# voletiv/mcvd-pytorch

Measured on AMD Instinct MI355X. Metric: sampled frames/sec (whole node), SMMNIST 64x64 DDPM 100-step, higher is better.
Workload: dtype f32-equivalent: f32 storage and accumulation; 58 of 58 3x3 convs, 41 of 41 1x1 convs and the attention products (head dims 32..128) as SIX bf16 piece products of operands split EXACTLY into three bf16 pieces (all 24 bits, fp32 exponent range, less than one fp32 rounding per product; tests/test_gpu_p

## Files before the change

mcvd_pytorch_amd/csrc/build.py:

```python
import argparse
import concurrent.futures as cf
import glob
import os
import subprocess
import sys

HERE = os.path.dirname(os.path.abspath(__file__))
PKG = os.path.dirname(HERE)
ROOT = os.path.dirname(PKG)
OBJ = os.path.join(HERE, "build")
LIB = os.path.join(PKG, "libmcvd_hip.so")
HIPCC = os.environ.get("HIPCC", "/opt/rocm/bin/hipcc")
FLAGS = ["--offload-arch=gfx950", "-O3", "-std=c++17", "-fPIC", "-Wall", "-Wno-unused-function",
         "-I", os.path.join(ROOT, "include")]
WINO_OBJS = ("conv_wino.o", "conv_wino3.o", "conv_wino2h.o", "conv_wino3p.o")
HOST_ONLY_FLAGS = {"model.cpp": ["-ffp-contract=off"], "api.cpp": ["-ffp-contract=off"],
                   "sampler.cpp": ["-ffp-contract=off"],
                   "dsm.cpp": ["-ffp-contract=off"],
                   "lpips.cpp": ["-ffp-contract=off"]}


def sources():
    return sorted(glob.glob(os.path.join(HERE, "*.cpp")) + glob.glob(os.path.join(HERE, "kernels", "*.cpp")))


def headers():
    return (glob.glob(os.path.join(HERE, "*.h")) + glob.glob(os.path.join(HERE, "kernels", "*.h"))
            + glob.glob(os.path.join(ROOT, "include", "*.h")) + [os.path.abspath(__file__)])


def compile_one(src, force, diag=False):
    obj = os.path.join(OBJ + ("_diag" if diag else ""), os.path.basename(src)[:-4] + ".o")
    newest_dep = max(os.path.getmtime(p) for p in [src] + headers())
    if not force and os.path.exists(obj) and os.path.getmtime(obj) >= newest_dep:
        return obj, None
    cmd = [HIPCC] + FLAGS + (["-DMCVD_DIAG"] if diag else []) + HOST_ONLY_FLAGS.get(os.path.basename(src), []) + ["-c", src, "-o", obj]
    r = subprocess.run(cmd, capture_output=True, text=True)
    if r.returncode != 0:
        raise RuntimeError("hipcc failed: %s\n%s" % (" ".join(cmd), r.stderr))
    return obj, r.stderr.strip()


def build(force=False, jobs=None, verbose=True, diag=False):
    lib = os.path.join(PKG, "libmcvd_hip_diag.so") if diag else LIB
    os.makedirs(OBJ + ("_diag" if diag else ""), exist_ok=True)
    srcs = sources()
    objs, rebuilt, wino_rebuilt = [], 0, False
    with cf.ThreadPoolExecutor(max_workers=jobs or os.cpu_count()) as ex:
        for obj, log in ex.map(lambda s: compile_one(s, force, diag), srcs):
            objs.append(obj)
            if log is not None:
                rebuilt += 1
                wino_rebuilt |= os.path.basename(obj) in WINO_OBJS
                if log and verbose:
                    print(log, file=sys.stderr)
    relink = rebuilt or not os.path.exists(lib) or force
    stamp = os.path.join(OBJ + ("_diag" if diag else ""), "wino_isa.ok")
    newest_wino = max(os.path.getmtime(os.path.join(OBJ + ("_diag" if diag else ""), o)) for o in WINO_OBJS)
    checked = os.path.exists(stamp) and os.path.getmtime(stamp) >= newest_wino
    if wino_rebuilt or (relink and not checked) or not checked:
        r = subprocess.run([sys.executable, os.path.join(ROOT, "tools", "check_wino_isa.py")] + (["--diag"] if diag else []),
                           capture_output=True, text=True)
        if r.returncode != 0:
            for o in WINO_OBJS:
                try:
                    os.remove(os.path.join(OBJ + ("_diag" if diag else ""), o))
                except OSError:
                    pass
            raise RuntimeError("Winograd kernels: generated code violates the asm-load invariants\n" + r.stderr)
        open(stamp, "w").write(r.stdout)
        if verbose:
            print(r.stdout.strip())
    if relink:
        cmd = [HIPCC, "--offload-arch=gfx950", "-shared", "-fPIC", "-o", lib] + objs + ["-ldl"]
        r = subprocess.run(cmd, capture_output=True, text=True)
        if r.returncode != 0:
            raise RuntimeError("link failed: %s\n%s" % (" ".join(cmd), r.stderr))
    if relink:
        r = subprocess.run([sys.executable, os.path.join(ROOT, "tools", "check_vop3p_dual_read.py"), lib], capture_output=True, text=True)
        if r.returncode != 0:
            os.remove(lib)
            raise RuntimeError("the library contains the gfx950 co-residency erratum form (write the affine with fma_unpacked, common.h)\n" + r.stdout + r.stderr)
        if verbose:
            print(r.stdout.strip())
    if verbose:
        print("%s: %d/%d objects rebuilt -> %s" % (os.path.basename(lib), rebuilt, len(srcs), lib))
    return lib


if __name__ == "__main__":
    ap = argparse.ArgumentParser()
    ap.add_argument("--force", action="store_true")
    ap.add_argument("-j", type=int, default=None)
    ap.add_argument("--diag", action="store_true", help="build libmcvd_hip_diag.so (-DMCVD_DIAG) instead")
    a = ap.parse_args()
    build(force=a.force, jobs=a.j, diag=a.diag)
```

mcvd_pytorch_amd/csrc/kernels/conv1x1_h2.cpp:

```cpp
#include <stdlib.h>

#include "../common.h"
#include "pieces.h"

namespace mcvd {

typedef float f32x16 __attribute__((ext_vector_type(16)));
typedef float f32x2 __attribute__((ext_vector_type(2)));
typedef unsigned u32x4 __attribute__((ext_vector_type(4)));

__device__ __forceinline__ float silu_q(float v) { return v * __builtin_amdgcn_rcpf(1.0f + __expf(-v)); }

constexpr int Q1_PT = 128;
constexpr int Q1_CK = 16;
constexpr int Q1_NB = 4;
constexpr int Q1_MAXIMG = 4;

template <int NP, int COT, int PRO, int EXP = 0, bool KV = false, bool IM = false>
__global__ __launch_bounds__(256, 2) void conv1x1_h2_kernel(ConvArgs a, int ptiles, int nct) {
    typedef Pieces<NP> PX;
    constexpr int PT = Q1_PT, CK = Q1_CK, NB = Q1_NB, BCO = 32 * COT;
    constexpr int PPR = PT / 4;
    constexpr int RPS = 256 / PPR;
    constexpr int XSZ = CK * PT;
    constexpr int WDW = COT * NP * 256;
    constexpr int WPC = WDW / 4;
    constexpr int MAXX = XSZ / 4 / 256;
    constexpr int MAXW = (WPC + 255) / 256;
    constexpr int G = (IM ? 0 : MAXX) + MAXW;
    static_assert(MAXX * 256 * 4 == XSZ && WPC % 64 == 0, "DMA rounds");
    extern __shared__ __attribute__((aligned(16))) float smem[];
    unsigned* sW = reinterpret_cast<unsigned*>(smem);
    float* sX = smem + NB * WDW;
    float* sC = sX + (IM ? 0 : NB * XSZ);

    const int tid = threadIdx.x, lane = tid & 63, wave = tid >> 6, l31 = lane & 31, half = lane >> 5;
    const int xcd = blockIdx.x & 7, slot = blockIdx.x >> 3;
    const int ptile = (slot / nct) * 8 + xcd, ctile = slot - (slot / nct) * nct;
    if (ptile >= ptiles) return;
    const int co0 = ctile * BCO;
    const int HW = a.H * a.W, Cin = a.Cin;
    const long NPX = (long)a.B * HW;
    const long gp0 = (long)ptile * PT;
    const int NS = a.CoutP / 32;

    long xg = gp0 + (tid % PPR) * 4;
    if (xg > NPX - 4) xg = NPX - 4;
    const int xb = (int)(xg / HW), xp = (int)(xg - (long)xb * HW);
    const int x_ci = tid / PPR;
    const int voff0 = (xb * a.C0 + x_ci) * HW + xp;
    const int voff1 = (xb * a.C1 + x_ci) * HW + xp;

    const unsigned* wbase = reinterpret_cast<const unsigned*>(NP == 2 ? a.wph : a.wpb) + PX::HDR + (long)ctile * COT * (NP * 256);
    const int wave_u = __builtin_amdgcn_readfirstlane(wave);
    int w_goff[MAXW], w_lds[MAXW];
#pragma unroll
    for (int s = 0; s < MAXW; ++s) {
        const int q0 = (s * 256 + wave_u * 64) % WPC;
        w_lds[s] = q0 * 4;
        w_goff[s] = (q0 + lane) * 4;
    }

    const int b_first = (int)(gp0 / HW);
    const int nimg = HW >= PT ? 1 : PT / HW;
    if (PRO != 0) {
        const int ppi = Cin >> 1;
        for (int q0 = 0; q0 < nimg * ppi; q0 += 256) {
            const int q = q0 + tid;
            if (q < nimg * ppi) {
                const int im = q / ppi, w = q - im * ppi;
                __builtin_amdgcn_global_load_lds(
                    (const __attribute__((address_space(1))) void*)(a.coef + ((long)min(b_first + im, a.B - 1) * Cin) * 2 + w * 4),
                    (__attribute__((address_space(3))) void*)(sC + (q0 + wave * 64) * 4), 16, 0, 0);
            }
        }
    }
    const int my_img = HW >= PT ? 0 : (wave * 32) / HW;
    const int x_lane = wave * 32 + l31 + half * PT;

#define Q1_DMA(ch)                                                                                              \
    {                                                                                                           \
        const int cb = (ch) * CK;                                                                               \
        const unsigned* wsrc = wbase + (long)(ch) * NS * (NP * 256);                                                  \
        unsigned* wdst = sW + ((ch) & (NB - 1)) * WDW;                                                          \
        _Pragma("unroll") for (int s = 0; s < MAXW; ++s)                                                        \
            __builtin_amdgcn_global_load_lds(                                                                   \
                (const __attribute__((address_space(1))) void*)(wsrc + w_goff[s]),                              \
                (__attribute__((address_space(3))) void*)(wdst + w_lds[s]), 16, 0, 0);                          \
        if constexpr (!IM) {                                                                                    \
            const bool second = cb >= a.C0;                                                                     \
            const float* xsrc = second ? a.x1 + (long)(cb - a.C0) * HW : a.x0 + (long)cb * HW;                  \
            const int voff = second ? voff1 : voff0;                                                            \
            float* xdst = sX + ((ch) & (NB - 1)) * XSZ;                                                         \
            _Pragma("unroll") for (int s = 0; s < MAXX; ++s)                                                    \
                __builtin_amdgcn_global_load_lds(                                                               \
                    (const __attribute__((address_space(1))) void*)(xsrc + (long)s * RPS * HW + voff),          \
                    (__attribute__((address_space(3))) void*)(xdst + (s * 256 + wave * 64) * 4), 16, 0, 0);     \
        }                                                                                                       \
    }

    f32x16 acc[COT];
#pragma unroll
    for (int ct = 0; ct < COT; ++ct)
#pragma unroll
        for (int r = 0; r < 16; ++r) acc[ct][r] = 0.0f;

    const bool rec = a.dbg != nullptr && wave == 0;
    unsigned long long tk0 = 0, tk1 = 0, tk2 = 0, rt0 = 0;
    if (rec) { rt0 = __builtin_amdgcn_s_memrealtime(); tk0 = __builtin_amdgcn_s_memtime(); }

    const int nchunks = Cin / CK;
    Q1_DMA(0);
    if (nchunks > 1) Q1_DMA(1);
    if (nchunks > 2) Q1_DMA(2);
    float* sPatch = sX;
    const int im_W = a.W, im_PR = PT / (IM ? a.W : PT) + 2, im_PITCH = a.W + 8, im_Cc = a.C0 + a.C1;
    const int im_plane = im_PR * im_PITCH;
    int* sTab = reinterpret_cast<int*>(sPatch + (im_Cc + 1) * im_plane);
    int im_base = 0;
    if constexpr (IM) {
        typedef float f4 __attribute__((ext_vector_type(4)));
        const int y0 = (int)((gp0 - (long)b_first * HW) / im_W);
        const int w4 = im_W >> 2, lw4 = 31 - __builtin_clz(w4);
        const int rows = (im_Cc + 1) * im_PR;
        for (int u0 = 0; u0 < rows * w4; u0 += 2 * 256) {
            f4 v[2];
            int dst[2];
#pragma unroll
            for (int j = 0; j < 2; ++j) {
                const int u = u0 + j * 256 + tid;
                const int row = u >> lw4, q = u & (w4 - 1);
                const int c = row / im_PR, ry = row - c * im_PR;
                const int yy = y0 - 1 + ry;
                v[j] = f4{0.0f, 0.0f, 0.0f, 0.0f};
                dst[j] = u < rows * w4 ? row * im_PITCH + 4 + 4 * q : -1;
                if (dst[j] >= 0 && c < im_Cc && yy >= 0 && yy < a.H)
                    v[j] = *reinterpret_cast<const f4*>(c < a.C0 ? a.x0 + (((long)b_first * a.C0 + c) * a.H + yy) * im_W + 4 * q
                                                                 : a.x1 + (((long)b_first * a.C1 + (c - a.C0)) * a.H + yy) * im_W + 4 * q);
            }
#pragma unroll
            for (int j = 0; j < 2; ++j)
                if (dst[j] >= 0) *reinterpret_cast<f4*>(sPatch + dst[j]) = v[j];
        }
        for (int u = tid; u < 2 * rows; u += 256)
            *reinterpret_cast<f4*>(sPatch + (u >> 1) * im_PITCH + (u & 1) * (im_W + 4)) = f4{0.0f, 0.0f, 0.0f, 0.0f};
        for (int kk = tid; kk < Cin; kk += 256) {
            const int c = kk / 9, t = kk - 9 * c;
            const int off = c < im_Cc ? c * im_plane + (t / 3) * im_PITCH + (t % 3) + 3 : im_Cc * im_plane + 4;
            sTab[(kk >> 4) * 16 + (kk & 1) * 8 + ((kk & 15) >> 1)] = off;
        }
        const int p = wave * 32 + l31;
        im_base = (p / im_W) * im_PITCH + (p % im_W);
    }
    if (rec) tk1 = __builtin_amdgcn_s_memtime();
#define Q1_STAGE(k, BV, CF)                                                                                     \
    {                                                                                                           \
        const int after = nchunks - 1 - (k);                                                                    \
        if (after >= 2) asm volatile("s_waitcnt vmcnt(%0)" :: "n"(2 * G) : "memory");                           \
        else if (after == 1) asm volatile("s_waitcnt vmcnt(%0)" :: "n"(G) : "memory");                          \
        else asm volatile("s_waitcnt vmcnt(0)" ::: "memory");                                                   \
        if (!(EXP & 8)) {       \
            asm volatile("" ::: "memory");                                                                      \
            __builtin_amdgcn_s_waitcnt(0xC07F);                                                  \
            __builtin_amdgcn_s_barrier();                                                                       \
            asm volatile("" ::: "memory");                                                                      \
        }                                                                                                       \
        if ((k) + 3 < nchunks && !(EXP & 1)) Q1_DMA((k) + 3);                                                   \
        const float* sXc = sX + ((k) & (NB - 1)) * XSZ + x_lane;        \
        const float* sCb = sC + ((long)my_img * Cin + (k) * CK) * 2 + half * 2;                                 \
        if constexpr (IM) {      \
            const u32x4* tp = reinterpret_cast<const u32x4*>(sTab + (k) * 16 + half * 8);                       \
            const u32x4 t0 = tp[0], t1 = tp[1];                                                                 \
            const float* pb = sPatch + im_base;                                                                 \
            BV[0] = pb[t0[0]]; BV[1] = pb[t0[1]]; BV[2] = pb[t0[2]]; BV[3] = pb[t0[3]];                         \
            BV[4] = pb[t1[0]]; BV[5] = pb[t1[1]]; BV[6] = pb[t1[2]]; BV[7] = pb[t1[3]];                         \
        } else {                                                                                                \
        _Pragma("unroll") for (int e = 0; e < 8; ++e) {          \
            BV[e] = sXc[2 * e * PT];                                                                            \
            if (PRO != 0) CF[e] = *reinterpret_cast<const f32x2*>(sCb + 4 * e);                                 \
        }                                                                                                       \
        }                                                                                                       \
        __builtin_amdgcn_sched_barrier(0);                                                                      \
    }
#define Q1_READ_AW(k, AW)                                                                                       \
    {                                                                                                           \
        const u32x4* sWc = reinterpret_cast<const u32x4*>(sW + ((k) & (NB - 1)) * WDW) + lane;                  \
        _Pragma("unroll") for (int ct = 0; ct < COT; ++ct)                                                      \
            _Pragma("unroll") for (int p = 0; p < NP; ++p) AW[ct][p] = sWc[(ct * NP + p) * 64];                 \
    }
#define Q1_PREP(BV, CF, BP)                                                                                     \
    if (EXP & 4) { _Pragma("unroll") for (int p = 0; p < NP; ++p) _Pragma("unroll") for (int j = 0; j < 4; ++j) BP[p][j] = __builtin_bit_cast(unsigned, BV[2 * j]); } else \
    {                                                                                                           \
        _Pragma("unroll") for (int e = 0; e < 8; ++e) {                                                         \
            if (PRO != 0) {      \
                asm("v_fma_f32 %0, %1, %2, %3" : "=v"(BV[e]) : "v"(BV[e]), "v"(CF[e].x), "v"(CF[e].y));         \
                if (PRO == 2) BV[e] = silu_q(BV[e]);                                                            \
            }                                                                                                   \
            if (NP == 2) BV[e] *= PX::ACT_SCALE;                                                                \
        }                                                                                                       \
        _Pragma("unroll") for (int j = 0; j < 4; ++j) {                                                         \
            unsigned w[NP];                                                                                     \
            PX::template split<false>(BV[2 * j], BV[2 * j + 1], w);                                             \
            _Pragma("unroll") for (int p = 0; p < NP; ++p) BP[p][j] = w[p];                                     \
        }                                                                                                       \
    }
#define Q1_MMA(AW, BP)                                                                                          \
    if (EXP & 2) { _Pragma("unroll") for (int ct = 0; ct < COT; ++ct) acc[ct][0] += __builtin_bit_cast(float, AW[ct][0][0] ^ BP[0][1] ^ AW[ct][NP - 1][2] ^ BP[NP - 1][3]); } else \
    {                                                                                                           \
        _Pragma("unroll") for (int k = 0; k < PX::NPROD; ++k)                                                   \
            _Pragma("unroll") for (int ct = 0; ct < COT; ++ct) acc[ct] = PX::mfma(AW[ct][PX::PA(k)], BP[PX::PB(k)], acc[ct]); \
    }
#define Q1_STEP(k, BPC, BPN)                                                                                    \
    {                                                                                                           \
        Q1_STAGE((k) + 1, bv, cf)                                                                               \
        Q1_MMA(aw, BPC)                                                                                         \
        Q1_PREP(bv, cf, BPN)                                                                                    \
         \
        if (!(EXP & 16)) {                                                                                      \
             \
            __builtin_amdgcn_sched_group_barrier(0x008, 3, 0);                                                  \
            _Pragma("unroll") for (int i_ = 3; i_ < PX::NPROD * COT; ++i_) {                                    \
                __builtin_amdgcn_sched_group_barrier(0x002, NVS, 0);                                            \
                __builtin_amdgcn_sched_group_barrier(0x008, 1, 0);                                              \
            }                                                                                                   \
            _Pragma("unroll") for (int p_ = 0; p_ < NP; ++p_) asm volatile("" : "+v"(BPN[p_]));                 \
        }                                                                                                       \
        Q1_READ_AW((k) + 1, aw)                                                                                 \
    }
    constexpr int NVS = (PRO == 2 ? 120 : PRO == 1 ? 76 : 64) / (PX::NPROD * COT > 3 ? PX::NPROD * COT - 3 : 1) + 1;
    {
        float bv[8];
        f32x2 cf[8];
        u32x4 aw[COT][NP], bpA[NP], bpB[NP];
        Q1_STAGE(0, bv, cf)
        Q1_READ_AW(0, aw)
        Q1_PREP(bv, cf, bpA)
        int ch = 0;
        for (; ch + 2 < nchunks; ch += 2) {
            Q1_STEP(ch, bpA, bpB)
            Q1_STEP(ch + 1, bpB, bpA)
        }
        if (ch + 1 < nchunks) {
            Q1_STEP(ch, bpA, bpB)
            Q1_MMA(aw, bpB)
        } else {
            Q1_MMA(aw, bpA)
        }
    }
#undef Q1_STEP
#undef Q1_STAGE
#undef Q1_READ_AW
#undef Q1_PREP
#undef Q1_MMA
#undef Q1_DMA
    if (rec) tk2 = __builtin_amdgcn_s_memtime();

    const float inv = NP == 2 ? a.wph[2] * (1.0f / PX::ACT_SCALE) : 1.0f;
    float* sO = smem;
    constexpr int OPT = PT + 4;
    typedef float f32x4 __attribute__((ext_vector_type(4)));
    const int px4 = tid & 31, cr = tid >> 5;
    const long gp = gp0 + px4 * 4;
    const bool valid = gp < NPX;
    const long gpc = valid ? gp : 0;
    const int ob = (int)(gpc / HW), op = (int)(gpc - (long)ob * HW);
    const long obase = (long)ob * a.Cout * HW + op;
    float e_bias[BCO / 8];
    f32x4 e_res[BCO / 8];
#pragma unroll
    for (int k = 0; k < BCO / 8; ++k) {
        const int co = co0 + cr + 8 * k;
        e_bias[k] = a.bias[co];
        e_res[k] = f32x4{0.0f, 0.0f, 0.0f, 0.0f};
        if (a.res) e_res[k] = *reinterpret_cast<const f32x4*>(a.res + obase + (long)min(co, a.Cout - 1) * HW);
    }
    asm volatile("s_waitcnt lgkmcnt(0)\n\ts_barrier" ::: "memory");
#pragma unroll
    for (int ct = 0; ct < COT; ++ct)
#pragma unroll
        for (int r = 0; r < 16; ++r)
            sO[(ct * 32 + (r & 3) + 8 * (r >> 2) + 4 * half) * OPT + wave * 32 + l31] = acc[ct][r] * inv;
    asm volatile("s_waitcnt lgkmcnt(0)\n\ts_barrier" ::: "memory");
    bool kv_tile[COT];
#pragma unroll
    for (int ct = 0; ct < COT; ++ct) kv_tile[ct] = false;
    if constexpr (KV) {
        const int Cq = a.kv_C, D = a.kv_D, DT = D >> 5, heads = Cq / D, ntl = HW >> 5;
        unsigned* img = reinterpret_cast<unsigned*>(a.kv_img);
#pragma unroll
        for (int ct = 0; ct < COT; ++ct) {
            const int cs = co0 + ct * 32;
            const int which = cs / Cq;
            if (which != 1 && which != 2) continue;
            kv_tile[ct] = true;
            const int within = cs - which * Cq, head = within / D, ch0 = within - head * D;
#pragma unroll
            for (int rnd = 0; rnd < 2; ++rnd) {
                const int item = rnd * 256 + tid;
                if (which == 1) {
                    const int rp = item >> 5, p4 = item & 31;
                    const int st_l = rp >> 3, j = (rp >> 1) & 3, h = rp & 1;
                    const int rl = ct * 32 + 16 * st_l + 4 * j + h;
                    const long g = gp0 + p4 * 4;
                    if (g < NPX) {
                        const int bb = (int)(g / HW), pix = (int)(g - (long)bb * HW);
                        const f32x4 v0 = *reinterpret_cast<const f32x4*>(sO + rl * OPT + p4 * 4) + a.bias[co0 + rl];
                        const f32x4 v1 = *reinterpret_cast<const f32x4*>(sO + (rl + 2) * OPT + p4 * 4) + a.bias[co0 + rl + 2];
                        unsigned w[4][3];
#pragma unroll
                        for (int i4 = 0; i4 < 4; ++i4) Pieces<3>::template split<false>(v0[i4], v1[i4], w[i4]);
                        const int st = (ch0 >> 4) + st_l;
                        unsigned* d1 = img + ((long)(bb * heads + head) * ntl + (pix >> 5)) * (3072 * DT) + (st * 3 * 4 + j) * 64 + h * 32 + (pix & 31);
#pragma unroll
                        for (int pc = 0; pc < 3; ++pc) *reinterpret_cast<u32x4*>(d1 + pc * 256) = u32x4{w[0][pc], w[1][pc], w[2][pc], w[3][pc]};
                    }
                } else {
                    const int m = item & 31, grp = item >> 5;
                    const int tt = grp >> 2, s2 = (grp >> 1) & 1, h = grp & 1;
                    const int kb = 16 * s2 + 4 * h;
                    const long g = gp0 + tt * 32;
                    if (g < NPX) {
                        const int bb = (int)(g / HW), pix = (int)(g - (long)bb * HW);
                        const int rl = ct * 32 + m;
                        const float bs = a.bias[co0 + rl];
                        const f32x4 v0 = *reinterpret_cast<const f32x4*>(sO + rl * OPT + tt * 32 + kb) + bs;
                        const f32x4 v1 = *reinterpret_cast<const f32x4*>(sO + rl * OPT + tt * 32 + kb + 8) + bs;
                        unsigned wa[3], wb[3], wc[3], wd[3];
                        Pieces<3>::template split<false>(v0[0], v0[1], wa);
                        Pieces<3>::template split<false>(v0[2], v0[3], wb);
                        Pieces<3>::template split<false>(v1[0], v1[1], wc);
                        Pieces<3>::template split<false>(v1[2], v1[3], wd);
                        unsigned* d1 = img + ((long)(bb * heads + head) * ntl + (pix >> 5)) * (3072 * DT) + 1536 * DT +
                                       ((((ch0 >> 5) * 2 + s2) * 3) * 64 + h * 32 + m) * 4;
#pragma unroll
                        for (int pc = 0; pc < 3; ++pc) *reinterpret_cast<u32x4*>(d1 + pc * 256) = u32x4{wa[pc], wb[pc], wc[pc], wd[pc]};
                    }
                }
            }
        }
    }
    {
#pragma unroll
        for (int k = 0; k < BCO / 8; ++k) {
            if (KV && kv_tile[k >> 2]) continue;
            const int cl = cr + 8 * k, co = co0 + cl;
            f32x4 v = *reinterpret_cast<const f32x4*>(sO + cl * OPT + px4 * 4);
            v = (v + e_bias[k] + e_res[k]) * a.out_scale;
            if (valid && co < a.Cout) *reinterpret_cast<f32x4*>(a.y + obase + (long)co * HW) = v;
            if (a.stats && (HW >= PT || HW == 64)) {
                const bool g16 = HW == 64;
                float pil;
                {
                    const int pv = __builtin_bit_cast(int, v[0]);
                    const int s0 = __builtin_amdgcn_readlane(pv, 0), s1 = __builtin_amdgcn_readlane(pv, 16);
                    const int s2 = __builtin_amdgcn_readlane(pv, 32), s3 = __builtin_amdgcn_readlane(pv, 48);
                    pil = __builtin_bit_cast(float, (lane & 32) ? ((g16 && (lane & 16)) ? s3 : s2) : ((g16 && (lane & 16)) ? s1 : s0));
                }
                const float d0 = v[0] - pil, d1 = v[1] - pil, d2 = v[2] - pil, d3 = v[3] - pil;
                float sm = (d0 + d1) + (d2 + d3);
                float qm = (d0 * d0 + d1 * d1) + (d2 * d2 + d3 * d3);
#define Q1_MERGE(CTRL, ROWMASK)                                                                                     \
                {                                                                                                   \
                    sm += __builtin_bit_cast(float, __builtin_amdgcn_update_dpp(0, __builtin_bit_cast(int, sm), CTRL, ROWMASK, 0xf, false)); \
                    qm += __builtin_bit_cast(float, __builtin_amdgcn_update_dpp(0, __builtin_bit_cast(int, qm), CTRL, ROWMASK, 0xf, false)); \
                }
                Q1_MERGE(0xB1, 0xf)
                Q1_MERGE(0x4E, 0xf)
                Q1_MERGE(0x124, 0xf)
                Q1_MERGE(0x128, 0xf)
                float sm2 = sm, qm2 = qm;
                sm2 += __builtin_bit_cast(float, __builtin_amdgcn_update_dpp(0, __builtin_bit_cast(int, sm), 0x142, 0xa, 0xf, false));
                qm2 += __builtin_bit_cast(float, __builtin_amdgcn_update_dpp(0, __builtin_bit_cast(int, qm), 0x142, 0xa, 0xf, false));
#undef Q1_MERGE
                if (!g16) { sm = sm2; qm = qm2; }
                const bool writer = g16 ? (px4 & 15) == 0 : px4 == 31;
                if (writer && valid && co < a.Cout) {
                    const float npix = g16 ? 64.0f : 128.0f;
                    const int np = g16 ? 1 : HW >> 7, pidx = g16 ? 0 : op >> 7;
                    float* q = a.stats + (((long)ob * a.Cout + co) * np + pidx) * 2;
                    q[0] = sm + npix * pil;
                    q[1] = fmaxf(qm - sm * sm / npix, 0.0f);
                }
            }
        }
    }
    if (rec) {
        const unsigned long long now = __builtin_amdgcn_s_memtime();
        if (lane == 0) {
            unsigned hwid, xcc;
            asm volatile("s_getreg_b32 %0, hwreg(HW_REG_HW_ID)" : "=s"(hwid));
            asm volatile("s_getreg_b32 %0, hwreg(HW_REG_XCC_ID)" : "=s"(xcc));
            unsigned long long* d = a.dbg + (long)blockIdx.x * 8;
            d[0] = tk1 - tk0; d[1] = tk2 - tk1; d[2] = rt0; d[3] = __builtin_amdgcn_s_memrealtime();
            d[4] = ((unsigned long long)xcc << 32) | hwid;
            d[5] = now - tk2; d[6] = (unsigned long long)nchunks; d[7] = now - tk0;
        }
    }
}

static size_t q1_lds_bytes(int np, int cot, int Cin, int HW, int im_cc = 0, int W = 0) {
    const int nimg = HW >= Q1_PT ? 1 : Q1_PT / HW;
    const size_t pix = im_cc > 0 ? (size_t)((im_cc + 1) * (Q1_PT / W + 2) * (W + 8) + Cin) : (size_t)Q1_NB * Q1_CK * Q1_PT + (size_t)nimg * Cin * 2;
    const size_t loop = ((size_t)Q1_NB * (cot * np * 256) + pix) * sizeof(float);
    const size_t epi = (size_t)(32 * cot) * (Q1_PT + 4) * sizeof(float);
    return loop > epi ? loop : epi;
}

bool conv1x1_h2_supported(const ConvArgs& a, int cot, int np) {
    const int HW = a.H * a.W;
    if (np != 2 && np != 3) return false;
    if (a.ks != 1 || !(np == 2 ? a.wph : a.wpb) || HW % 32 != 0 || cot < 1 || cot > 4 || (a.CoutP / 32) % cot != 0) return false;
    if (a.im2col) {
        return np == 3 && !a.coef && !a.act && !a.kv_img && a.W >= 8 && a.W <= Q1_PT && (a.W & (a.W - 1)) == 0 && HW % Q1_PT == 0 && a.Cin % Q1_CK == 0 &&
               a.Cin == a.CinP && a.Cin >= 9 * (a.C0 + a.C1) && (long)a.B * (a.C0 > a.C1 ? a.C0 : a.C1) * HW < (1L << 31) &&
               q1_lds_bytes(np, cot, a.Cin, HW, a.C0 + a.C1, a.W) <= 80 * 1024;
    }
    if (!(HW % Q1_PT == 0 || (HW < Q1_PT && Q1_PT % HW == 0 && Q1_PT / HW <= Q1_MAXIMG))) return false;
    if (a.Cin % Q1_CK != 0 || a.CinP % Q1_CK != 0) return false;
    if (a.C1 > 0 && a.C0 % Q1_CK != 0) return false;
    if ((long)a.B * (a.C0 > a.C1 ? a.C0 : a.C1) * HW >= (1L << 31)) return false;
    if (a.act && !a.coef) return false;
    return q1_lds_bytes(np, cot, a.Cin, HW) <= 80 * 1024;
}

template <int NP, int COT>
static int q1_launch(const ConvArgs& a, hipStream_t s) {
    const int HW = a.H * a.W;
    const long NPX = (long)a.B * HW;
    const int ptiles = (int)((NPX + Q1_PT - 1) / Q1_PT);
    const int nct = a.CoutP / (32 * COT);
    const size_t lds = q1_lds_bytes(NP, COT, a.Cin, HW, a.im2col ? a.C0 + a.C1 : 0, a.W);
    const dim3 grid(((ptiles + 7) / 8) * 8 * nct);
    if constexpr (NP == 3) {
        if (a.im2col) {
            static PerDeviceOnce raised_im;
            if (lds > 48 * 1024 && raised_im.first_use()) {
                MCVD_HIP_CHECK(hipFuncSetAttribute(reinterpret_cast<const void*>(&conv1x1_h2_kernel<3, COT, 0, 0, false, true>), hipFuncAttributeMaxDynamicSharedMemorySize, 160 * 1024));
                raised_im.done();
            }
            hipLaunchKernelGGL((conv1x1_h2_kernel<3, COT, 0, 0, false, true>), grid, dim3(256), lds, s, a, ptiles, nct);
            MCVD_HIP_CHECK(hipGetLastError());
            return 0;
        }
    }
    static PerDeviceOnce raised;
    if (lds > 48 * 1024 && raised.first_use()) {
        MCVD_HIP_CHECK(hipFuncSetAttribute(reinterpret_cast<const void*>(&conv1x1_h2_kernel<NP, COT, 0>), hipFuncAttributeMaxDynamicSharedMemorySize, 160 * 1024));
        MCVD_HIP_CHECK(hipFuncSetAttribute(reinterpret_cast<const void*>(&conv1x1_h2_kernel<NP, COT, 1>), hipFuncAttributeMaxDynamicSharedMemorySize, 160 * 1024));
        MCVD_HIP_CHECK(hipFuncSetAttribute(reinterpret_cast<const void*>(&conv1x1_h2_kernel<NP, COT, 2>), hipFuncAttributeMaxDynamicSharedMemorySize, 160 * 1024));
        if constexpr (NP == 3)
            MCVD_HIP_CHECK(hipFuncSetAttribute(reinterpret_cast<const void*>(&conv1x1_h2_kernel<3, COT, 1, 0, true>), hipFuncAttributeMaxDynamicSharedMemorySize, 160 * 1024));
        raised.done();
    }
#ifdef MCVD_DIAG
    {
        const char* es = getenv("MCVD_Q1_EXP");
        const int e = es ? atoi(es) : 0;
        if (e != 0 && NP == 3 && COT == 3) {
            static PerDeviceOnce raised2;
            if (raised2.first_use()) {
                (void)hipFuncSetAttribute(reinterpret_cast<const void*>(&conv1x1_h2_kernel<3, 3, 1, 1>), hipFuncAttributeMaxDynamicSharedMemorySize, 160 * 1024);
                (void)hipFuncSetAttribute(reinterpret_cast<const void*>(&conv1x1_h2_kernel<3, 3, 1, 2>), hipFuncAttributeMaxDynamicSharedMemorySize, 160 * 1024);
                (void)hipFuncSetAttribute(reinterpret_cast<const void*>(&conv1x1_h2_kernel<3, 3, 1, 4>), hipFuncAttributeMaxDynamicSharedMemorySize, 160 * 1024);
                (void)hipFuncSetAttribute(reinterpret_cast<const void*>(&conv1x1_h2_kernel<3, 3, 1, 6>), hipFuncAttributeMaxDynamicSharedMemorySize, 160 * 1024);
                (void)hipFuncSetAttribute(reinterpret_cast<const void*>(&conv1x1_h2_kernel<3, 3, 1, 7>), hipFuncAttributeMaxDynamicSharedMemorySize, 160 * 1024);
                (void)hipFuncSetAttribute(reinterpret_cast<const void*>(&conv1x1_h2_kernel<3, 3, 1, 15>), hipFuncAttributeMaxDynamicSharedMemorySize, 160 * 1024);
                (void)hipFuncSetAttribute(reinterpret_cast<const void*>(&conv1x1_h2_kernel<3, 3, 1, 16>), hipFuncAttributeMaxDynamicSharedMemorySize, 160 * 1024);
                raised2.done();
            }
            switch (e) {
                case 1: hipLaunchKernelGGL((conv1x1_h2_kernel<3, 3, 1, 1>), grid, dim3(256), lds, s, a, ptiles, nct); break;
                case 2: hipLaunchKernelGGL((conv1x1_h2_kernel<3, 3, 1, 2>), grid, dim3(256), lds, s, a, ptiles, nct); break;
                case 4: hipLaunchKernelGGL((conv1x1_h2_kernel<3, 3, 1, 4>), grid, dim3(256), lds, s, a, ptiles, nct); break;
                case 6: hipLaunchKernelGGL((conv1x1_h2_kernel<3, 3, 1, 6>), grid, dim3(256), lds, s, a, ptiles, nct); break;
                case 7: hipLaunchKernelGGL((conv1x1_h2_kernel<3, 3, 1, 7>), grid, dim3(256), lds, s, a, ptiles, nct); break;
                case 16: hipLaunchKernelGGL((conv1x1_h2_kernel<3, 3, 1, 16>), grid, dim3(256), lds, s, a, ptiles, nct); break;
                default: hipLaunchKernelGGL((conv1x1_h2_kernel<3, 3, 1, 15>), grid, dim3(256), lds, s, a, ptiles, nct); break;
            }
            MCVD_HIP_CHECK(hipGetLastError());
            return 0;
        }
    }
    if constexpr (NP == 3) {
        static const bool noprio = getenv("MCVD_Q1_NOPRIO") && atoi(getenv("MCVD_Q1_NOPRIO")) != 0;
        if (noprio) {
            static PerDeviceOnce raised3;
            if (raised3.first_use()) {
                (void)hipFuncSetAttribute(reinterpret_cast<const void*>(&conv1x1_h2_kernel<NP, COT, 0, 16>), hipFuncAttributeMaxDynamicSharedMemorySize, 160 * 1024);
                (void)hipFuncSetAttribute(reinterpret_cast<const void*>(&conv1x1_h2_kernel<NP, COT, 1, 16>), hipFuncAttributeMaxDynamicSharedMemorySize, 160 * 1024);
                (void)hipFuncSetAttribute(reinterpret_cast<const void*>(&conv1x1_h2_kernel<NP, COT, 2, 16>), hipFuncAttributeMaxDynamicSharedMemorySize, 160 * 1024);
                raised3.done();
            }
            if (!a.coef) hipLaunchKernelGGL((conv1x1_h2_kernel<NP, COT, 0, 16>), grid, dim3(256), lds, s, a, ptiles, nct);
            else if (!a.act) hipLaunchKernelGGL((conv1x1_h2_kernel<NP, COT, 1, 16>), grid, dim3(256), lds, s, a, ptiles, nct);
            else hipLaunchKernelGGL((conv1x1_h2_kernel<NP, COT, 2, 16>), grid, dim3(256), lds, s, a, ptiles, nct);
            MCVD_HIP_CHECK(hipGetLastError());
            return 0;
        }
    }
#endif
    if constexpr (NP == 3) {
        if (a.kv_img && a.coef && !a.act) {
            hipLaunchKernelGGL((conv1x1_h2_kernel<3, COT, 1, 0, true>), grid, dim3(256), lds, s, a, ptiles, nct);
            MCVD_HIP_CHECK(hipGetLastError());
            return 0;
        }
    }
    if (!a.coef)
        hipLaunchKernelGGL((conv1x1_h2_kernel<NP, COT, 0>), grid, dim3(256), lds, s, a, ptiles, nct);
    else if (!a.act)
        hipLaunchKernelGGL((conv1x1_h2_kernel<NP, COT, 1>), grid, dim3(256), lds, s, a, ptiles, nct);
    else
        hipLaunchKernelGGL((conv1x1_h2_kernel<NP, COT, 2>), grid, dim3(256), lds, s, a, ptiles, nct);
    MCVD_HIP_CHECK(hipGetLastError());
    return 0;
}

template <int NP>
static int q1_launch_cot(const ConvArgs& a, int cot, hipStream_t s) {
    switch (cot) {
        case 1: return q1_launch<NP, 1>(a, s);
        case 2: return q1_launch<NP, 2>(a, s);
        case 3: return q1_launch<NP, 3>(a, s);
        default: return q1_launch<NP, 4>(a, s);
    }
}

bool conv1x1_h2_kv_supported(const ConvArgs& a, int cot) {
    return a.kv_img && a.kv_C > 0 && a.Cout == 3 * a.kv_C && a.kv_D % 32 == 0 && a.kv_C % a.kv_D == 0 && a.coef && !a.act && !a.res && a.out_scale == 1.0f &&
           !a.stats && conv1x1_h2_supported(a, cot, 3);
}

int launch_conv1x1_h2(const ConvArgs& a, int cot, hipStream_t s, int np) {
    MCVD_REQUIRE(!a.kv_img || (np == 3 && conv1x1_h2_kv_supported(a, cot)), "conv1x1 split-operand GEMM: K / V piece images requested for a launch that cannot write them");
    MCVD_REQUIRE(conv1x1_h2_supported(a, cot, np), "conv1x1 split-operand GEMM: unsupported (np=%d ks=%d H=%d W=%d Cin=%d C0=%d cot=%d, weight pieces %s)",
                 np, a.ks, a.H, a.W, a.Cin, a.C0, cot, (np == 2 ? a.wph : a.wpb) ? "present" : "missing");
    const int rc = np == 2 ? q1_launch_cot<2>(a, cot, s) : q1_launch_cot<3>(a, cot, s);
    const int HW = a.H * a.W;
    if (rc == 0 && a.stats && (HW >= Q1_PT || HW == 64)) set_last_conv_stats_np(HW >= Q1_PT ? HW / Q1_PT : 1);
    return rc;
}

__global__ void q1_absmax_kernel(const float* w, long n, unsigned* hdr) {
    float m = 0.0f;
    for (long i = blockIdx.x * (long)blockDim.x + threadIdx.x; i < n; i += (long)gridDim.x * blockDim.x) m = fmaxf(m, fabsf(w[i]));
#pragma unroll
    for (int o = 32; o > 0; o >>= 1) m = fmaxf(m, __shfl_xor(m, o));
    if ((threadIdx.x & 63) == 0) atomicMax(hdr, __float_as_uint(m));
}

__global__ void pack_conv1x1_h2_kernel(const float* wp, float* wh, int CinP, int CoutP) {
    const float wmax = wh[0];
    int k = 0;
    (void)frexpf(wmax, &k);
    const int e = (wmax > 0.0f && wmax < 3.0e38f) ? min(max(14 - k, -60), 60) : 0;
    const float scale = ldexpf(1.0f, e);
    if (blockIdx.x == 0 && threadIdx.x == 0) { wh[1] = scale; wh[2] = ldexpf(1.0f, -e); }
    _Float16* dst = reinterpret_cast<_Float16*>(wh + Pieces<2>::HDR);
    const long n = (long)CinP * CoutP;
    const int NS = CoutP / 32;
    for (long i = blockIdx.x * (long)blockDim.x + threadIdx.x; i < n; i += (long)gridDim.x * blockDim.x) {
        const int co = (int)(i % CoutP), ci = (int)(i / CoutP);
        const float us = wp[i] * scale;
        const _Float16 h1 = (_Float16)us;
        const _Float16 h2 = (_Float16)(us - (float)h1);
        const int cc = ci & 15, h = cc & 1, el = cc >> 1, lane = h * 32 + (co & 31);
        const long o = (((long)(ci >> 4) * NS + (co >> 5)) * 2) * 512 + (lane * 4 + (el >> 1)) * 2 + (el & 1);
        dst[o] = h1;
        dst[o + 512] = h2;
    }
}

__global__ void pack_conv1x1_b3_kernel(const float* wp, unsigned short* dst, int CinP, int CoutP) {
    const long n = (long)CinP * CoutP;
    const int NS = CoutP / 32;
    for (long i = blockIdx.x * (long)blockDim.x + threadIdx.x; i < n; i += (long)gridDim.x * blockDim.x) {
        const int co = (int)(i % CoutP), ci = (int)(i / CoutP);
        const float u = wp[i];
        const unsigned short h1 = px_bf16_rne(u);
        const float r1 = u - px_bf16_f32(h1);
        const unsigned short h2 = px_bf16_rne(r1);
        const float r2 = r1 - px_bf16_f32(h2);
        const unsigned short h3 = px_bf16_rne(r2);
        const int cc = ci & 15, h = cc & 1, el = cc >> 1, lane = h * 32 + (co & 31);
        const long o = (((long)(ci >> 4) * NS + (co >> 5)) * 3) * 512 + (lane * 4 + (el >> 1)) * 2 + (el & 1);
        dst[o] = h1;
        dst[o + 512] = h2;
        dst[o + 1024] = h3;
    }
}

long conv1x1_h2_weight_floats(int CinP, int CoutP, int np) {
    return np == 2 ? Pieces<2>::HDR + (long)CinP * CoutP : (long)CinP * CoutP / 2 * 3;
}

int launch_pack_conv1x1_h2(const float* wp, float* wh, int CinP, int CoutP, hipStream_t s, int np) {
    MCVD_REQUIRE(CinP % 16 == 0 && CoutP % 32 == 0 && (np == 2 || np == 3), "pack_conv1x1_h2: CinP=%d CoutP=%d np=%d", CinP, CoutP, np);
    const long n = (long)CinP * CoutP;
    const int blocks = (int)((n + 255) / 256 > 4096 ? 4096 : (n + 255) / 256);
    if (np == 2) {
        hipLaunchKernelGGL(q1_absmax_kernel, dim3(blocks), dim3(256), 0, s, wp, n, reinterpret_cast<unsigned*>(wh));
        hipLaunchKernelGGL(pack_conv1x1_h2_kernel, dim3(blocks), dim3(256), 0, s, wp, wh, CinP, CoutP);
    } else {
        hipLaunchKernelGGL(pack_conv1x1_b3_kernel, dim3(blocks), dim3(256), 0, s, wp, reinterpret_cast<unsigned short*>(wh), CinP, CoutP);
    }
    MCVD_HIP_CHECK(hipGetLastError());
    return 0;
// ... 4 lines not shown
```

mcvd_pytorch_amd/csrc/model.cpp:

```cpp
#include "model.h"
#include "conv_kernels.h"

#include <math.h>
#include <stdarg.h>
#include <stdio.h>
#include <string.h>

#include <algorithm>
#include <tuple>

namespace mcvd {

static thread_local char g_err[1024] = "";
void set_error(const char* fmt, ...) {
    va_list ap;
    va_start(ap, fmt);
    vsnprintf(g_err, sizeof(g_err), fmt, ap);
    va_end(ap);
}
const char* get_error() { return g_err; }

static int gn_groups(int ch) {
    int g = std::min(ch / 4, 32);
    while (g > 1 && ch % g != 0) --g;
// ... 967 lines not shown
                a.cot = cot;
                a.shape_hint = shape;
                if (launch_conv_mfma(a, s)) return 0;
                MCVD_HIP_CHECK(hipEventRecord(e0, s));
                for (int r = 0; r < 3; ++r)
                    if (int rc = launch_conv_mfma(a, s)) return rc;
                MCVD_HIP_CHECK(hipEventRecord(e1, s));
                MCVD_HIP_CHECK(hipEventSynchronize(e1));
                float ms = 0.f;
                MCVD_HIP_CHECK(hipEventElapsedTime(&ms, e0, e1));
                if (ms < best_ms) { best_ms = ms; choice = {shape, cot}; }
                return 0;
            };
            auto offer = [&](int id, int cot) -> int {
                a.cot = cot;
                return conv_kernel_usable(id, a) ? time_candidate(id, cot) : 0;
            };
            const int cots[2] = {op.cot, 1};
            for (int ci = 0; ci < (op.cot == 1 ? 1 : 2); ++ci) {
                for (int shape = CK_TILE256; shape <= CK_WINO; ++shape) {
                    if (spade_fused && conv_kernel_usable(CK_WINO, a) && shape != CK_WINO) continue;
                    if (shape == CK_TILE_SPLITK && (op.ks != 3 || !ctx->conv_wdma)) continue;
                    if (shape == CK_WINO && (ci > 0 || !ctx->winograd || !conv_kernel_usable(CK_WINO, a))) continue;
                    const int bpx = shape == CK_TILE256 ? 256 : shape == CK_TILE128 ? 128 : 64;
                    const bool fits = bpx % op.W == 0 && (bpx / op.W <= op.H ? op.H % (bpx / op.W) == 0 : (bpx / op.W) % op.H == 0);
                    if (shape != CK_WINO && !fits) continue;
                    if (int rc = time_candidate(shape, cots[ci])) return rc;
                }
            }
            a.cot = op.cot;
            if (op.alt_kind && !spade_fused && op.gb.kind == REF_NONE) {
                ConvArgs t = a;
                t.shape_hint = op.alt_kind;
                t.stats = (ctx->gn_stats && op.stats.kind != REF_NONE) ? resolve(op.stats, scratch_io, scratch_io, scratch_io, B) : nullptr;
                float* buf = resolve(op.alt_buf, scratch_io, scratch_io, scratch_io, B);
                for (int c = 4; c >= 1; --c) {
                    t.cot = c;
                    if (!gemm_form_usable(op, t)) break;
                    if (gemm_form_args(op, t, buf).cot != c) continue;
                    if (launch_gemm_form(op, t, buf, s)) continue;
                    MCVD_HIP_CHECK(hipEventRecord(e0, s));
                    for (int r = 0; r < 3; ++r)
                        if (int rc = launch_gemm_form(op, t, buf, s)) return rc;
                    MCVD_HIP_CHECK(hipEventRecord(e1, s));
                    MCVD_HIP_CHECK(hipEventSynchronize(e1));
                    float ms = 0.f;
                    MCVD_HIP_CHECK(hipEventElapsedTime(&ms, e0, e1));
                    if (ms < best_ms) { best_ms = ms; choice = {op.alt_kind, c}; }
                }
            }
            if (op.ks == 3 && ctx->winograd)
                if (int rc = offer(CK_WINO_K2, op.cot)) return rc;
            if (op.ks == 3 && ctx->winograd && ctx->bf16x3 && !spade_fused) {
                for (int id : {CK_WINO3, CK_WINO3_K2, CK_WINO3P, CK_WINO3P_K2})
                    if (int rc = offer(id, op.cot)) return rc;
                const bool g8 = op.H == 8 && op.W == 8;
                const long pairs = (g8 ? (B + 1) / 2 : (long)B * (op.H / 8) * (op.W / 16)) * (op.CoutP / (32 * conv_wino_cout_tile(op.Cout)));
                if (2 * pairs < 1024) {
                    for (int id : {CK_WINO3_K4, CK_WINO3P_K4})
                        if (int rc = offer(id, op.cot)) return rc;
                    if (4 * pairs < 1024)
                        if (int rc = offer(CK_WINO3_K8, op.cot)) return rc;
                }
            }
            const bool f16_ok = ctx->f16x2 && a.coef != nullptr;
            if (op.ks == 3 && ctx->winograd && f16_ok && !spade_fused)
                for (int id : {CK_WINO2H, CK_WINO2H_K2})
                    if (int rc = offer(id, op.cot)) return rc;
            if (op.ks == 1 && ctx->conv_dma1) {
                static const int g1_cots[] = {2, 1, 3, 4, 6, 9};
                for (int id : {CK_DMA1, CK_DMA1_CK32}) {
                    int tried = 0;
                    for (int c : g1_cots) {
                        a.cot = c;
                        if ((op.CoutP / 32) % c != 0 || tried >= 3 || !conv_kernel_usable(id, a)) continue;
                        ++tried;
                        if (int rc = time_candidate(id, c)) return rc;
                    }
                }
                if (f16_ok)
                    for (int c = 4; c >= 1; --c)
                        if (int rc = offer(CK_GEMM1_F16X2, c)) return rc;
                if (ctx->bf16x3)
                    for (int c = 4; c >= 1; --c)
                        if (int rc = offer(CK_GEMM1_BF16X3, c)) return rc;
                if (int rc = offer(CK_DMA1_PX64, 1)) return rc;
                if ((op.CoutP / 32) % 2 == 0)
                    if (int rc = offer(CK_DMA1_PX64, 2)) return rc;
            }
            it = best.emplace(k, choice).first;
        }
        tuned_shape[i] = it->second.first;
        tuned_cot[i] = it->second.second;
    }
    (void)hipEventDestroy(e0);
    (void)hipEventDestroy(e1);
    tuned_B = B;
    ++epoch;
    return 0;
}

void mcvd_model::sync_tuning_options() {
    const int sig = (ctx->winograd ? 1 : 0) | (ctx->conv_dma1 ? 2 : 0) | (ctx->bf16x3 ? 4 : 0) | (ctx->f16x2 ? 8 : 0) |
                    (ctx->spade_fuse ? 16 : 0) | (ctx->conv_wdma ? 32 : 0);
    if (sig != tuned_sig) {
        if (tuned_sig >= 0) { tuned_cache.clear(); tuned_B = 0; }
        tuned_sig = sig;
    }
}

int mcvd_model::ensure_f16x2_weights() {
    if (packed_h_valid || packed_h_floats == 0) return 0;
    hipStream_t s = ctx->stream;
    if (!packed_h) MCVD_HIP_CHECK(hipMalloc((void**)&packed_h, (size_t)packed_h_floats * sizeof(float)));
    MCVD_HIP_CHECK(hipMemsetAsync(packed_h, 0, (size_t)packed_h_floats * sizeof(float), s));
    for (const ConvPack& p : packs) {
        if (p.wph < 0) continue;
        if (p.ks == 3) {
            const ParamInfo& w = params[find_param(p.weights[0].c_str())];
            if (int rc = launch_pack_wino2h_weight(blob + w.off, packed_h + p.wph, p.Cout_each, p.Cin, p.CinP, p.CoutP, s)) return rc;
        } else {
            if (int rc = launch_pack_conv1x1_h2(packed + p.wp, packed_h + p.wph, p.CinP, p.CoutP, s, 2)) return rc;
        }
    }
    MCVD_HIP_CHECK(hipStreamSynchronize(s));
    packed_h_valid = true;
    ++epoch;
    return 0;
}

int mcvd_model::ensure_ksplit(int B) {
    size_t need = 0;
    const std::vector<int>* table = nullptr;
    auto it = tuned_cache.find(B);
    if (it != tuned_cache.end() && it->second.first.size() == ops.size()) table = &it->second.first;
    for (size_t i = 0; i < ops.size(); ++i) {
        const Op& op = ops[i];
        if (!(op.kind == OP_CONV && op.ks == 3 && op.wpw >= 0 && op.H * op.W <= 256)) continue;
        int parts = 2;
        const bool g8 = op.H == 8 && op.W == 8;
        const long pairs = (g8 ? (B + 1) / 2 : (long)B * (op.H / 8) * (op.W / 16)) * (op.CoutP / (32 * conv_wino_cout_tile(op.Cout)));
        if (ctx->autotune && !table && tuned_B != B && 2 * pairs < 1024) parts = 4 * pairs < 1024 ? 8 : 4;
        auto deepen = [&](int shape) { parts = std::max(parts, k_parts(shape)); };
        deepen(ctx->conv_shape);
        if (table) deepen((*table)[i]);
        if (tuned_B == B && i < tuned_shape.size()) deepen(tuned_shape[i]);
        need = std::max(need, (size_t)parts * B * op.Cout * op.H * op.W);
    }
    if (need <= ksplit_floats) return 0;
    MCVD_HIP_CHECK(hipStreamSynchronize(ctx->stream));
    if (ksplit_buf) MCVD_HIP_CHECK(hipFree(ksplit_buf));
    ksplit_buf = nullptr;
    ksplit_floats = 0;
    MCVD_HIP_CHECK(hipMalloc((void**)&ksplit_buf, need * sizeof(float)));
    ksplit_floats = need;
    ++epoch;
    return 0;
}

int mcvd_model::prepare_B(int B) {
    if (int rc = ensure_workspace(B)) return rc;
    sync_tuning_options();
    if (int rc = ensure_ksplit(B)) return rc;
    const bool forced_h = pieces(ctx->conv_shape) == 2 || ctx->conv_shape1 == CK_GEMM1_F16X2;
    if (ctx->f16x2 || forced_h)
        if (int rc = ensure_f16x2_weights()) return rc;
    if (!ctx->naive_conv && tuned_B != B) {
// ... 180 lines not shown
```

Measured before the change: 264.6.

## Load 1x1 conv weight pieces straight to registers instead of staging through LDS

The split-operand 1x1 GEMM kernel now loads its weight piece fragments directly from global memory into double-buffered registers with inline-asm dwordx4 loads, two chunks ahead. This replaces the LDS DMA staging and the LDS reads. The vmcnt waits are reworked to count the weight loads separately from the activation DMA, and LDS use drops by the weight buffers, which could raise occupancy. In exchange it needs more VGPRs, so COT=4 is dropped for three pieces, and a new build-time ISA check is added to guard the ordering of the asm loads.

```diff
diff --git a/mcvd_pytorch_amd/csrc/build.py b/mcvd_pytorch_amd/csrc/build.py
--- a/mcvd_pytorch_amd/csrc/build.py
+++ b/mcvd_pytorch_amd/csrc/build.py
@@ -71,6 +71,17 @@
         open(stamp, "w").write(r.stdout)
         if verbose:
             print(r.stdout.strip())
+    q1_obj = os.path.join(OBJ + ("_diag" if diag else ""), "conv1x1_h2.o")
+    q1_stamp = os.path.join(OBJ + ("_diag" if diag else ""), "conv1x1_isa.ok")
+    if not (os.path.exists(q1_stamp) and os.path.getmtime(q1_stamp) >= os.path.getmtime(q1_obj)):
+        r = subprocess.run([sys.executable, os.path.join(ROOT, "tools", "check_conv1x1_isa.py")] + (["--diag"] if diag else []),
+                           capture_output=True, text=True)
+        if r.returncode != 0:
+            os.remove(q1_obj)
+            raise RuntimeError("conv1x1_h2_kernel: generated code violates the asm-load invariants\n" + r.stderr)
+        open(q1_stamp, "w").write(r.stdout)
+        if verbose:
+            print(r.stdout.strip())
     if relink:
         cmd = [HIPCC, "--offload-arch=gfx950", "-shared", "-fPIC", "-o", lib] + objs + ["-ldl"]
         r = subprocess.run(cmd, capture_output=True, text=True)
diff --git a/mcvd_pytorch_amd/csrc/kernels/conv1x1_h2.cpp b/mcvd_pytorch_amd/csrc/kernels/conv1x1_h2.cpp
--- a/mcvd_pytorch_amd/csrc/kernels/conv1x1_h2.cpp
+++ b/mcvd_pytorch_amd/csrc/kernels/conv1x1_h2.cpp
@@ -10,6 +10,18 @@
 typedef unsigned u32x4 __attribute__((ext_vector_type(4)));
 
 __device__ __forceinline__ float silu_q(float v) { return v * __builtin_amdgcn_rcpf(1.0f + __expf(-v)); }
+
+template <int I>
+__device__ __forceinline__ void q1_load_a(u32x4& d, unsigned voff, const unsigned* chunk) {
+    asm volatile("global_load_dwordx4 %0, %1, %2 offset:%3" : "=&v"(d) : "v"(voff), "s"(chunk + (I >> 2) * 1024), "n"((I & 3) * 1024) : "memory");
+}
+template <int NP, int I, int N>
+__device__ __forceinline__ void q1_load_as(u32x4 (*aw)[NP], unsigned voff, const unsigned* chunk) {
+    if constexpr (I < N) {
+        q1_load_a<I>(aw[I / NP][I % NP], voff, chunk);
+        q1_load_as<NP, I + 1, N>(aw, voff, chunk);
+    }
+}
 
 constexpr int Q1_PT = 128;
 constexpr int Q1_CK = 16;
@@ -23,15 +35,12 @@
     constexpr int PPR = PT / 4;
     constexpr int RPS = 256 / PPR;
     constexpr int XSZ = CK * PT;
-    constexpr int WDW = COT * NP * 256;
-    constexpr int WPC = WDW / 4;
+    constexpr int AWN = COT * NP;
     constexpr int MAXX = XSZ / 4 / 256;
-    constexpr int MAXW = (WPC + 255) / 256;
-    constexpr int G = (IM ? 0 : MAXX) + MAXW;
-    static_assert(MAXX * 256 * 4 == XSZ && WPC % 64 == 0, "DMA rounds");
+    constexpr int GX = IM ? 0 : MAXX;
+    static_assert(MAXX * 256 * 4 == XSZ && 3 * AWN + 2 * MAXX < 64, "DMA rounds, vmcnt range");
     extern __shared__ __attribute__((aligned(16))) float smem[];
-    unsigned* sW = reinterpret_cast<unsigned*>(smem);
-    float* sX = smem + NB * WDW;
+    float* sX = smem;
     float* sC = sX + (IM ? 0 : NB * XSZ);
 
     const int tid = threadIdx.x, lane = tid & 63, wave = tid >> 6, l31 = lane & 31, half = lane >> 5;
@@ -52,14 +61,10 @@
     const int voff1 = (xb * a.C1 + x_ci) * HW + xp;
 
     const unsigned* wbase = reinterpret_cast<const unsigned*>(NP == 2 ? a.wph : a.wpb) + PX::HDR + (long)ctile * COT * (NP * 256);
-    const int wave_u = __builtin_amdgcn_readfirstlane(wave);
-    int w_goff[MAXW], w_lds[MAXW];
-#pragma unroll
-    for (int s = 0; s < MAXW; ++s) {
-        const int q0 = (s * 256 + wave_u * 64) % WPC;
-        w_lds[s] = q0 * 4;
-        w_goff[s] = (q0 + lane) * 4;
-    }
+    const int nchunks = Cin / CK;
+    const unsigned aw_voff = lane * 16;
+#define Q1_LOAD_AW(k, AW) q1_load_as<NP, 0, AWN>(AW, aw_voff, wbase + (long)(k) * NS * (NP * 256));
+    u32x4 awA[COT][NP], awB[COT][NP];
 
     const int b_first = (int)(gp0 / HW);
     const int nimg = HW >= PT ? 1 : PT / HW;
@@ -81,12 +86,6 @@
 #define Q1_DMA(ch)                                                                                              \
     {                                                                                                           \
         const int cb = (ch) * CK;                                                                               \
-        const unsigned* wsrc = wbase + (long)(ch) * NS * (NP * 256);                                                  \
-        unsigned* wdst = sW + ((ch) & (NB - 1)) * WDW;                                                          \
-        _Pragma("unroll") for (int s = 0; s < MAXW; ++s)                                                        \
-            __builtin_amdgcn_global_load_lds(                                                                   \
-                (const __attribute__((address_space(1))) void*)(wsrc + w_goff[s]),                              \
-                (__attribute__((address_space(3))) void*)(wdst + w_lds[s]), 16, 0, 0);                          \
         if constexpr (!IM) {                                                                                    \
             const bool second = cb >= a.C0;                                                                     \
             const float* xsrc = second ? a.x1 + (long)(cb - a.C0) * HW : a.x0 + (long)cb * HW;                  \
@@ -109,10 +108,10 @@
     unsigned long long tk0 = 0, tk1 = 0, tk2 = 0, rt0 = 0;
     if (rec) { rt0 = __builtin_amdgcn_s_memrealtime(); tk0 = __builtin_amdgcn_s_memtime(); }
 
-    const int nchunks = Cin / CK;
     Q1_DMA(0);
     if (nchunks > 1) Q1_DMA(1);
     if (nchunks > 2) Q1_DMA(2);
+    Q1_LOAD_AW(0, awA)
     float* sPatch = sX;
     const int im_W = a.W, im_PR = PT / (IM ? a.W : PT) + 2, im_PITCH = a.W + 8, im_Cc = a.C0 + a.C1;
     const int im_plane = im_PR * im_PITCH;
@@ -153,12 +152,30 @@
         im_base = (p / im_W) * im_PITCH + (p % im_W);
     }
     if (rec) tk1 = __builtin_amdgcn_s_memtime();
+#define Q1_WAIT(NA, NX) asm volatile("s_waitcnt vmcnt(%0)" :: "n"((NA) * AWN + (NX) * GX) : "memory");
+#define Q1_WAIT_AW1(NA, NX, BP)                                                                                 \
+    {                                                                                                           \
+        if constexpr (NP == 2) asm volatile("s_waitcnt vmcnt(%2)" : "+v"(BP[0]), "+v"(BP[1]) : "n"((NA) * AWN + (NX) * GX) : "memory"); \
+        else asm volatile("s_waitcnt vmcnt(%3)" : "+v"(BP[0]), "+v"(BP[1]), "+v"(BP[NP - 1]) : "n"((NA) * AWN + (NX) * GX) : "memory"); \
+    }
+#define Q1_WAIT_AW(k, BP)                                                                                       \
+    {                                                                                                           \
+        const int after_ = nchunks - 1 - (k);                                                                   \
+        if (after_ >= 4) Q1_WAIT_AW1(1, 2, BP) else if (after_ == 3) Q1_WAIT_AW1(1, 1, BP)                      \
+        else if (after_ >= 1) Q1_WAIT_AW1(1, 0, BP) else Q1_WAIT_AW1(0, 0, BP)                                  \
+    }
 #define Q1_STAGE(k, BV, CF)                                                                                     \
     {                                                                                                           \
-        const int after = nchunks - 1 - (k);                                                                    \
-        if (after >= 2) asm volatile("s_waitcnt vmcnt(%0)" :: "n"(2 * G) : "memory");                           \
-        else if (after == 1) asm volatile("s_waitcnt vmcnt(%0)" :: "n"(G) : "memory");                          \
-        else asm volatile("s_waitcnt vmcnt(0)" ::: "memory");                                                   \
+        if constexpr (!IM) {                                                                                    \
+            const int after = nchunks - 1 - (k);                                                                \
+            if ((k) >= 2) {                                                                                     \
+                if (after >= 2) Q1_WAIT(3, 2) else if (after == 1) Q1_WAIT(3, 1) else Q1_WAIT(3, 0)             \
+            } else if ((k) == 1) {                                                                              \
+                if (after >= 2) Q1_WAIT(2, 2) else if (after == 1) Q1_WAIT(2, 1) else Q1_WAIT(2, 0)             \
+            } else {                                                                                            \
+                if (after >= 2) Q1_WAIT(1, 2) else if (after == 1) Q1_WAIT(1, 1) else Q1_WAIT(1, 0)             \
+            }                                                                                                   \
+        }                                                                                                       \
         if (!(EXP & 8)) {       \
             asm volatile("" ::: "memory");                                                                      \
             __builtin_amdgcn_s_waitcnt(0xC07F);                                                  \
@@ -182,12 +199,6 @@
         }                                                                                                       \
         __builtin_amdgcn_sched_barrier(0);                                                                      \
     }
-#define Q1_READ_AW(k, AW)                                                                                       \
-    {                                                                                                           \
-        const u32x4* sWc = reinterpret_cast<const u32x4*>(sW + ((k) & (NB - 1)) * WDW) + lane;                  \
-        _Pragma("unroll") for (int ct = 0; ct < COT; ++ct)                                                      \
-            _Pragma("unroll") for (int p = 0; p < NP; ++p) AW[ct][p] = sWc[(ct * NP + p) * 64];                 \
-    }
 #define Q1_PREP(BV, CF, BP)                                                                                     \
     if (EXP & 4) { _Pragma("unroll") for (int p = 0; p < NP; ++p) _Pragma("unroll") for (int j = 0; j < 4; ++j) BP[p][j] = __builtin_bit_cast(unsigned, BV[2 * j]); } else \
     {                                                                                                           \
@@ -210,10 +221,11 @@
         _Pragma("unroll") for (int k = 0; k < PX::NPROD; ++k)                                                   \
             _Pragma("unroll") for (int ct = 0; ct < COT; ++ct) acc[ct] = PX::mfma(AW[ct][PX::PA(k)], BP[PX::PB(k)], acc[ct]); \
     }
-#define Q1_STEP(k, BPC, BPN)                                                                                    \
+#define Q1_STEP(k, AW, BPC, BPN, MORE)                                                                          \
     {                                                                                                           \
         Q1_STAGE((k) + 1, bv, cf)                                                                               \
-        Q1_MMA(aw, BPC)                                                                                         \
+        Q1_WAIT_AW(k, BPC)                                                                                      \
+        Q1_MMA(AW, BPC)                                                                                         \
         Q1_PREP(bv, cf, BPN)                                                                                    \
          \
         if (!(EXP & 16)) {                                                                                      \
@@ -225,31 +237,37 @@
             }                                                                                                   \
             _Pragma("unroll") for (int p_ = 0; p_ < NP; ++p_) asm volatile("" : "+v"(BPN[p_]));                 \
         }                                                                                                       \
-        Q1_READ_AW((k) + 1, aw)                                                                                 \
+        __builtin_amdgcn_sched_barrier(0);    \
+        if (MORE) Q1_LOAD_AW((k) + 2, AW)                                                                       \
     }
     constexpr int NVS = (PRO == 2 ? 120 : PRO == 1 ? 76 : 64) / (PX::NPROD * COT > 3 ? PX::NPROD * COT - 3 : 1) + 1;
     {
         float bv[8];
         f32x2 cf[8];
-        u32x4 aw[COT][NP], bpA[NP], bpB[NP];
+        u32x4 bpA[NP], bpB[NP];
         Q1_STAGE(0, bv, cf)
-        Q1_READ_AW(0, aw)
+        Q1_LOAD_AW(min(1, nchunks - 1), awB)
         Q1_PREP(bv, cf, bpA)
         int ch = 0;
         for (; ch + 2 < nchunks; ch += 2) {
-            Q1_STEP(ch, bpA, bpB)
-            Q1_STEP(ch + 1, bpB, bpA)
+            Q1_STEP(ch, awA, bpA, bpB, true)
+            Q1_STEP(ch + 1, awB, bpB, bpA, ch + 3 < nchunks)
         }
         if (ch + 1 < nchunks) {
-            Q1_STEP(ch, bpA, bpB)
-            Q1_MMA(aw, bpB)
+            Q1_STEP(ch, awA, bpA, bpB, false)
+            Q1_WAIT_AW1(0, 0, bpB)
+            Q1_MMA(awB, bpB)
         } else {
-            Q1_MMA(aw, bpA)
+            Q1_WAIT_AW1(0, 0, bpA)
+            Q1_MMA(awA, bpA)
         }
     }
 #undef Q1_STEP
 #undef Q1_STAGE
-#undef Q1_READ_AW
+#undef Q1_LOAD_AW
+#undef Q1_WAIT
+#undef Q1_WAIT_AW
+#undef Q1_WAIT_AW1
 #undef Q1_PREP
 #undef Q1_MMA
 #undef Q1_DMA
@@ -401,7 +419,7 @@
 static size_t q1_lds_bytes(int np, int cot, int Cin, int HW, int im_cc = 0, int W = 0) {
     const int nimg = HW >= Q1_PT ? 1 : Q1_PT / HW;
     const size_t pix = im_cc > 0 ? (size_t)((im_cc + 1) * (Q1_PT / W + 2) * (W + 8) + Cin) : (size_t)Q1_NB * Q1_CK * Q1_PT + (size_t)nimg * Cin * 2;
-    const size_t loop = ((size_t)Q1_NB * (cot * np * 256) + pix) * sizeof(float);
+    const size_t loop = pix * sizeof(float);
     const size_t epi = (size_t)(32 * cot) * (Q1_PT + 4) * sizeof(float);
     return loop > epi ? loop : epi;
 }
@@ -409,6 +427,7 @@
 bool conv1x1_h2_supported(const ConvArgs& a, int cot, int np) {
     const int HW = a.H * a.W;
     if (np != 2 && np != 3) return false;
+    if (np == 3 && cot > 3) return false;
     if (a.ks != 1 || !(np == 2 ? a.wph : a.wpb) || HW % 32 != 0 || cot < 1 || cot > 4 || (a.CoutP / 32) % cot != 0) return false;
     if (a.im2col) {
         return np == 3 && !a.coef && !a.act && !a.kv_img && a.W >= 8 && a.W <= Q1_PT && (a.W & (a.W - 1)) == 0 && HW % Q1_PT == 0 && a.Cin % Q1_CK == 0 &&
@@ -522,7 +541,9 @@
         case 1: return q1_launch<NP, 1>(a, s);
         case 2: return q1_launch<NP, 2>(a, s);
         case 3: return q1_launch<NP, 3>(a, s);
-        default: return q1_launch<NP, 4>(a, s);
+        default:
+            if constexpr (NP == 2) return q1_launch<NP, 4>(a, s);
+            return -1;
     }
 }
 
diff --git a/mcvd_pytorch_amd/csrc/model.cpp b/mcvd_pytorch_amd/csrc/model.cpp
--- a/mcvd_pytorch_amd/csrc/model.cpp
+++ b/mcvd_pytorch_amd/csrc/model.cpp
@@ -1073,7 +1073,7 @@
                     for (int c = 4; c >= 1; --c)
                         if (int rc = offer(CK_GEMM1_F16X2, c)) return rc;
                 if (ctx->bf16x3)
-                    for (int c = 4; c >= 1; --c)
+                    for (int c = 3; c >= 1; --c)
                         if (int rc = offer(CK_GEMM1_BF16X3, c)) return rc;
                 if (int rc = offer(CK_DMA1_PX64, 1)) return rc;
                 if ((op.CoutP / 32) % 2 == 0)
```

Result: no change. 265.1 (median of 2 runs) (+0.2%).
